# TinyMPC/TinyMPC

Hardware: AMD Instinct MI355X
Metric: QP solves/sec (+ ADMM iters/sec), 64k-batch quadrotor hover (higher is better)
Workload: dtype f64; 1 GPU; quadrotor_hovering (nx=12, nu=4, N=10), 65536 identical instances per GPU, closed-loop MPC steps from a cold start (BASELINE configs[1]); batch_per_gpu=65536, total_batch=65536, parallelism=batch-sharded x1, mpc_steps_per_launch=8, stats_exchange=none (one rank), launcher=plain process

## Files before the change

tinympc_amd/csrc/admm_kernel.hip.h:

```cpp
#pragma once
#include <hip/hip_runtime.h>
#include <stdint.h>

namespace tinympc_amd {

enum : int {
    TAB_MB = 0,
    TAB_MF1 = 256,
    TAB_MF2 = 512,
    TAB_PT = 768,
    TAB_VEC = 1024,
    TAB_BOUNDS = 1024 + 16 * 16,
};
enum : int {
    VEC_CB = 0,
    VEC_CF = 1,
    VEC_QR = 2,
    VEC_SMASK = 3,
    VEC_NIM = 4,
    VEC_SOCFLAG = 5,
    VEC_CONE_BASE = 6,
    VEC_CONE_MU = 7,
    VEC_LINFLAG = 9,
    VEC_TLINFLAG = 10,
// ... 133 lines not shown
        ring1<0, NA>(a0, srcA, mA);
        ring1<NA, NB>(a0, srcB, mB);
        return a0;
    } else {
        double a0 = init, a1 = 0.0;
        ring<MODE, 0, NA>(a0, a1, srcA, mA);
        ring<MODE, NA, NB>(a0, a1, srcB, mB);
        return a0 + a1;
    }
}
template <int MODE, int COL0, int NCOL>
__device__ __forceinline__ double ring_sum(double init, double src, const double* m) {
    if constexpr (MODE == 2) {
        double a0 = init;
        ring1<COL0, NCOL>(a0, src, m);
        return a0;
    } else {
        double a0 = init, a1 = 0.0;
        ring<MODE, COL0, NCOL>(a0, a1, src, m);
        return a0 + a1;
    }
}
template <int MODE, int COL0, int NCOL>
__device__ __forceinline__ double ring_short(double init, double src, const double* m) {
    if constexpr (MODE == 1) return ring_sum<1, COL0, NCOL>(init, src, m);
    else { double a0 = init; ring1<COL0, NCOL>(a0, src, m); return a0; }
}


#define RINGH_LO(k, p) DPP_FMA("a0", "src", "m" #k, "%[c0]+" #k, "0x3")
#define RINGH_HI(k, p) DPP_FMA("a0", "src", "m" #k, "8+%[c0]+" #k, "0xc")
#define RINGH_CASE(K)                                                                                                                    \
    if constexpr (NCOL == K)                                                                                                             \
        asm("s_nop 1\n\t" DPP_REP(K, RINGH_LO) "s_nop 0\n\t" DPP_REP(K, RINGH_HI) : [a0] "+&v"(a0) : [src] "v"(src), [c0] "i"(COL0) DPP_REP(K, DPP_ROW_M));
template <int COL0, int NCOL>
__device__ __forceinline__ void ring1_half(double& a0, double src, const double* m) {
    static_assert(NCOL >= 1 && COL0 + NCOL <= 8, "one half row");
    RINGH_CASE(1) RINGH_CASE(2) RINGH_CASE(3) RINGH_CASE(4) RINGH_CASE(5) RINGH_CASE(6) RINGH_CASE(7) RINGH_CASE(8)
}


#if defined(TINYMPC_FUSED_NX) && defined(TINYMPC_FUSED_NU)
#define TINYMPC_FUSED 1
constexpr bool fused_shape(int na, int nb) { return na == TINYMPC_FUSED_NX && nb == TINYMPC_FUSED_NU; }
#define FUSED_ROW_OPERANDS [c0] "i"(TINYMPC_FUSED_NX) DPP_REP(TINYMPC_FUSED_NX, DPP_ROW_A) DPP_REP(TINYMPC_FUSED_NU, DPP_ROW_B)
#else
constexpr bool fused_shape(int, int) { return false; }
#endif
#define BWD_COL_A(k, p) DPP_FMA("acc", "sa", "a" #k, #k, "0xf")
#define BWD_COL_B(k, p) DPP_FMA("acc", "sb", "b" #k, "%[c0]+" #k, "0xf")
#define FWD_COL_A(k, p) DPP_FMA("t", "xi", "a" #k, #k, "0xf")
#define FWD_COL_B(k, p) DPP_FMA("xn", "t", "b" #k, "%[c0]+" #k, "0xf")
#define FWD_COL_B_INPLACE(k, p) DPP_FMA("t", "t", "b" #k, "%[c0]+" #k, "%[bm]")
template <int NA, int NB>
__device__ __forceinline__ void fused_backward_step(double& qlo, double& acc, double vn, double g, double qx, double rho, double smask, double cb,
                                                    double sa, double sb, const double* ma, const double* mb_) {
#ifdef TINYMPC_FUSED
    if constexpr (fused_shape(NA, NB)) {
        double tmp;
        asm("v_add_f64 %[tmp], %[vn], -%[g]\n\t"
            "v_fma_f64 %[qlo], -%[rho], %[tmp], %[qx]\n\t"
            "v_fma_f64 %[acc], %[qlo], %[smask], %[cb]\n\t"
            DPP_REP(TINYMPC_FUSED_NX, BWD_COL_A) DPP_REP(TINYMPC_FUSED_NU, BWD_COL_B)
            : [qlo] "=&v"(qlo), [acc] "=&v"(acc), [tmp] "=&v"(tmp)
            : [vn] "v"(vn), [g] "v"(g), [qx] "v"(qx), [rho] "v"(rho), [smask] "v"(smask), [cb] "v"(cb), [sa] "v"(sa), [sb] "v"(sb), FUSED_ROW_OPERANDS);
    }
#endif
}
template <int NA, int NB>
__device__ __forceinline__ void fused_backward_step_soc(double& qlo, double& acc, double vn, double g, double qx, double w, double rho,
                                                        double smask, double cb, double sa, double sb, const double* ma, const double* mb_) {
#ifdef TINYMPC_FUSED
    if constexpr (fused_shape(NA, NB)) {
        double tmp;
        asm("v_add_f64 %[tmp], %[vn], -%[g]\n\t"
            "v_fma_f64 %[qlo], -%[rho], %[tmp], %[qx]\n\t"
            "v_fma_f64 %[qlo], -%[rho], %[w], %[qlo]\n\t"
            "v_fma_f64 %[acc], %[qlo], %[smask], %[cb]\n\t"
            DPP_REP(TINYMPC_FUSED_NX, BWD_COL_A) DPP_REP(TINYMPC_FUSED_NU, BWD_COL_B)
            : [qlo] "=&v"(qlo), [acc] "=&v"(acc), [tmp] "=&v"(tmp)
            : [vn] "v"(vn), [g] "v"(g), [qx] "v"(qx), [rho] "v"(rho), [smask] "v"(smask), [cb] "v"(cb), [sa] "v"(sa), [sb] "v"(sb),
              [w] "v"(w), FUSED_ROW_OPERANDS);
    }
#endif
}
template <int NA, int NB, bool INPLACE = false>
__device__ __forceinline__ void fused_forward_step(double& tt, double& vn, double& t, double& xn, double xi, double g, double lo, double hi,
                                                   const double* ma, const double* mb_) {
#ifdef TINYMPC_FUSED
    if constexpr (fused_shape(NA, NB) && !(INPLACE && TINYMPC_FUSED_NX % 4 == 0)) {
        double vm;
        asm("v_add_f64 %[tt], %[xi], %[g]\n\t"
            "v_max_f64 %[vm], %[lo], %[tt]\n\t"
            DPP_REP(TINYMPC_FUSED_NX, FWD_COL_A)
            "v_min_f64 %[vn], %[hi], %[vm]\n\t"
            "v_mov_b64 %[xn], %[t]\n\t"
            DPP_REP(TINYMPC_FUSED_NU, FWD_COL_B)
            : [tt] "=&v"(tt), [vm] "=&v"(vm), [vn] "=&v"(vn), [xn] "=&v"(xn), [t] "+&v"(t)
            : [xi] "v"(xi), [g] "v"(g), [lo] "v"(lo), [hi] "v"(hi), FUSED_ROW_OPERANDS);
    }
    if constexpr (fused_shape(NA, NB) && INPLACE && TINYMPC_FUSED_NX % 4 == 0) {
        asm("v_add_f64 %[tt], %[xi], %[g]\n\t"
            DPP_REP(TINYMPC_FUSED_NX, FWD_COL_A)
            "v_max_f64 %[vn], %[lo], %[tt]\n\t"
            "v_min_f64 %[vn], %[hi], %[vn]\n\t"
            DPP_REP(TINYMPC_FUSED_NU, FWD_COL_B_INPLACE)
            : [tt] "=&v"(tt), [vn] "=&v"(vn), [t] "+&v"(t)
            : [xi] "v"(xi), [g] "v"(g), [lo] "v"(lo), [hi] "v"(hi), [bm] "i"((1 << (TINYMPC_FUSED_NX / 4)) - 1), FUSED_ROW_OPERANDS);
        xn = t;
    }
#endif
}
#if defined(TINYMPC_FUSED) && TINYMPC_FUSED_NX + TINYMPC_FUSED_NU <= 8
#define TINYMPC_FUSED_HALF 1
#endif
#define HBWD_COL_A_LO(k, p) DPP_FMA("acc", "sa", "a" #k, #k, "0x3")
#define HBWD_COL_A_HI(k, p) DPP_FMA("acc", "sa", "a" #k, "8+" #k, "0xc")
#define HBWD_COL_B_LO(k, p) DPP_FMA("acc", "sb", "b" #k, "%[c0]+" #k, "0x3")
#define HBWD_COL_B_HI(k, p) DPP_FMA("acc", "sb", "b" #k, "8+%[c0]+" #k, "0xc")
#define HFWD_COL_A_LO(k, p) DPP_FMA("t", "xi", "a" #k, #k, "0x3")
#define HFWD_COL_A_HI(k, p) DPP_FMA("t", "xi", "a" #k, "8+" #k, "0xc")
#define HFWD_COL_B_LO(k, p) DPP_FMA("xn", "t", "b" #k, "%[c0]+" #k, "0x3")
#define HFWD_COL_B_HI(k, p) DPP_FMA("xn", "t", "b" #k, "8+%[c0]+" #k, "0xc")
template <int NA, int NB>
__device__ __forceinline__ void fused_backward_step_half(double& qlo, double& acc, double& dnp, double& tmpn, double tmp, double vnn, double gn, double qx,
                                                         double rho, double smask, double cb, double nim, double cf, double sa, double sb,
                                                         const double* ma, const double* mb_) {
#ifdef TINYMPC_FUSED_HALF
    if constexpr (fused_shape(NA, NB)) {
        asm("v_fma_f64 %[qlo], -%[rho], %[tmp], %[qx]\n\t"
            "v_fma_f64 %[acc], %[qlo], %[smask], %[cb]\n\t"
            "v_fma_f64 %[dnp], %[sa], %[nim], %[cf]\n\t"
            DPP_REP(TINYMPC_FUSED_NX, HBWD_COL_A_LO) DPP_REP(TINYMPC_FUSED_NU, HBWD_COL_B_LO)
            "v_add_f64 %[tmpn], %[vnn], -%[gn]\n\t"
            DPP_REP(TINYMPC_FUSED_NX, HBWD_COL_A_HI) DPP_REP(TINYMPC_FUSED_NU, HBWD_COL_B_HI)
            : [qlo] "=&v"(qlo), [acc] "=&v"(acc), [dnp] "=&v"(dnp), [tmpn] "=&v"(tmpn)
            : [tmp] "v"(tmp), [vnn] "v"(vnn), [gn] "v"(gn), [qx] "v"(qx), [rho] "v"(rho), [smask] "v"(smask), [cb] "v"(cb),
              [nim] "v"(nim), [cf] "v"(cf), [sa] "v"(sa), [sb] "v"(sb), FUSED_ROW_OPERANDS);
    }
#endif
}
template <int NA, int NB>
__device__ __forceinline__ void fused_forward_step_half(double& tt, double& vn, double& t, double& xn, double& gnew, double xi, double g,
                                                        double lo, double hi, const double* ma, const double* mb_) {
#ifdef TINYMPC_FUSED_HALF
    if constexpr (fused_shape(NA, NB)) {
        double vm;
        asm("v_add_f64 %[tt], %[xi], %[g]\n\t"
            "v_max_f64 %[vm], %[lo], %[tt]\n\t"
            DPP_REP(TINYMPC_FUSED_NX, HFWD_COL_A_LO)
            "v_min_f64 %[vn], %[hi], %[vm]\n\t"
            DPP_REP(TINYMPC_FUSED_NX, HFWD_COL_A_HI)
            "v_mov_b64 %[xn], %[t]\n\t"
            "v_add_f64 %[gnew], %[tt], -%[vn]\n\t"
            DPP_REP(TINYMPC_FUSED_NU, HFWD_COL_B_LO)
            "s_nop 0\n\t"
            DPP_REP(TINYMPC_FUSED_NU, HFWD_COL_B_HI)
            : [tt] "=&v"(tt), [vm] "=&v"(vm), [vn] "=&v"(vn), [xn] "=&v"(xn), [t] "+&v"(t), [gnew] "=&v"(gnew)
            : [xi] "v"(xi), [g] "v"(g), [lo] "v"(lo), [hi] "v"(hi), FUSED_ROW_OPERANDS);
    }
#endif
}

__device__ __forceinline__ double vmax64(double a, double b) {
    double r;
    asm("v_max_f64 %0, %1, %2" : "=v"(r) : "v"(a), "v"(b));
    return r;
}
__device__ __forceinline__ double vmin64(double a, double b) {
    double r;
    asm("v_min_f64 %0, %1, %2" : "=v"(r) : "v"(a), "v"(b));
    return r;
}
__device__ __forceinline__ double pinned_sub64(double a, double b) {
    double r = a - b;
    asm volatile("" : "+v"(r));
    return r;
}
__device__ __forceinline__ double vclamp64(double lo, double hi, double t) {
    double r;
    asm("v_max_f64 %0, %1, %2\n\tv_min_f64 %0, %3, %0" : "=&v"(r) : "v"(lo), "v"(t), "v"(hi));
    return r;
}

__device__ __forceinline__ double vmax_abs64(double a, double b) {
    double r;
    asm("v_max_f64 %0, %1, |%2|" : "=v"(r) : "v"(a), "v"(b));
    return r;
}
template <bool OPAQUE>
// ... 114 lines not shown

#ifndef TINYMPC_LIN_WAVES
#define TINYMPC_LIN_WAVES 0
#endif
constexpr long solve_kernel_lin_lds(int nx, int nu, int n, bool soc, int lin, int kmax, bool ub) {
    const int nz = nx + nu, csl = (nz + 1) | 1, cs = (nz + 1) | 1;
    return 8L * (nx * 16 + (ub ? 2 : 2 * n * 16) + ((lin & 1) ? 3 * kmax * 16 + 2 * 4 * n * csl : 0) +
                 ((lin & 2) ? 3 * n * kmax * 16 + 2 * 4 * n * csl : 0) + (soc ? (4 * n + 1) * 3 * cs : 0));
}
constexpr bool solve_kernel_lin_planes(int nx, int nu, int n, bool soc, int lin, int kmax, bool ub) {
    return lin != 0 && solve_kernel_lin_lds(nx, nu, n, soc, lin, kmax, ub) <= 64 * 1024 - 512;
}
constexpr int solve_kernel_lin_waves(int nx, int nu, int n, bool soc, int lin, int kmax, bool ub) {
    if (!solve_kernel_lin_planes(nx, nu, n, soc, lin, kmax, ub)) return 1;
    if (TINYMPC_LIN_WAVES > 0) return TINYMPC_LIN_WAVES;
    return (solve_kernel_waves_per_simd(nx + nu, n, soc) == 2 && 8 * solve_kernel_lin_lds(nx, nu, n, soc, lin, kmax, ub) <= 158 * 1024) ? 2 : 1;
}
template <int NF, int KMAX_, int LW_, int LPI_>
__device__ __forceinline__ void project_halfspace_columns(const int t, const int inst, const int n, const int csl, const int R0, const int S0,
                                                          double* pv, double* pg, const double* tab, const int tab_stride, const int nk) {
#pragma clang fp contract(off)
    for (int c = S0 + t; c < n; c += LPI_) {
        const int at = (inst * n + c) * csl + R0;
        const double* tk = tab + c * tab_stride;
        double z[NF], t0[NF];
#pragma unroll
        for (int r = 0; r < NF; ++r) { z[r] = pv[at + r]; t0[r] = z[r]; }
        for (int k = 0; k < nk; ++k) {
            double cv = 0.0;
#pragma unroll
            for (int r = 0; r < NF; ++r) { const double pr = tk[k * LW_ + R0 + r] * z[r]; cv = cv + pr; }
            const double bk = tk[KMAX_ * LW_ + k * LW_ + R0];
            if (cv > bk) {
                const double dist = (cv - bk) / tk[2 * KMAX_ * LW_ + k * LW_ + R0];
#pragma unroll
                for (int r = 0; r < NF; ++r) { const double pr = dist * tk[k * LW_ + R0 + r]; z[r] = z[r] - pr; }
            }
        }
#pragma unroll
        for (int r = 0; r < NF; ++r) { pv[at + r] = z[r]; pg[at + r] = t0[r] - z[r]; }
    }
}

template <int NX, int NU, int N, bool SOC, bool DBG, int MODE, int LIN = 0, bool HET = false, int KMAX = LIN_KMAX, bool ADAPT = false, bool UB = false, bool HALF = false,
          bool PF = false>
__global__ __launch_bounds__(64)
__attribute__((amdgpu_waves_per_eu(LIN != 0 ? solve_kernel_lin_waves(NX, NU, N, SOC, LIN, KMAX, UB) : solve_kernel_waves_per_simd(NX + NU, N, SOC, false, ADAPT),
                                   LIN != 0 ? solve_kernel_lin_waves(NX, NU, N, SOC, LIN, KMAX, UB) : solve_kernel_waves_per_simd(NX + NU, N, SOC, false, ADAPT))))
void admm_solve_kernel(const SolveArgs P) {
    constexpr bool LS = (LIN & 1) != 0, LT = (LIN & 2) != 0;
    constexpr int NZ = NX + NU;
    static_assert(NZ <= 16, "one instance per 16-lane DPP row");
    constexpr bool FUSED = MODE == 2 && LIN == 0 && fused_shape(NX, NU);
    static_assert(!HALF || (NZ <= 8 && FUSED && !SOC && !DBG && !HET && !ADAPT), "half rows: nx+nu <= 8, the plain box kernel on its fused step blocks");
    static_assert(!PF || (MODE == 2 && !SOC && !DBG && LIN == 0 && !HET && !ADAPT), "prefetch form: the plain box kernel");
    constexpr int RL = HALF ? 8 : 16;
    constexpr int IPW = 64 / RL;
    constexpr int RECD = N * NZ;
    constexpr int PF_PIECES = (IPW * RECD * 8 + 1023) / 1024;
    constexpr int PF_ARR = PF_PIECES * 128;
    constexpr unsigned long long RMASK = HALF ? 0xFFull : 0xFFFFull;
    const int lane = threadIdx.x & 63;
    const int j = lane & (RL - 1);
    const int grp = lane / RL;
    const bool is_state = j < NX;
    const bool is_input = (j >= NX) && (j < NZ);

    __shared__ double sPt[NX * 16];
    __shared__ double sLo[UB ? 1 : N * 16];
    __shared__ double sHi[UB ? 1 : N * 16];
    __shared__ double sLin[LS ? 3 * KMAX * 16 : 1];
    __shared__ double sTLin[LT ? 3 * N * KMAX * 16 : 1];
#ifndef TINYMPC_SOC_PD
#define TINYMPC_SOC_PD 2
#endif
    constexpr int SPD = TINYMPC_SOC_PD, SPR = SPD + 1;
    constexpr int CS = SOC ? ((NZ + 1) | 1) : 1;
    constexpr int SLOT_D = 3 * CS;
    constexpr int PL_GC = CS, PL_VC = 2 * CS;
    __shared__ double sC[SOC ? (4 * N + 1) * SLOT_D : 1];
    __shared__ double sP[ADAPT ? 4 * NX * NX : 1];
    constexpr int AKC = NX > NU ? NX : NU;
    constexpr bool HA = HET && ADAPT;
    __shared__ double sTab[(ADAPT && !HET) ? 3 * 16 * AKC : 1];
    __shared__ double sDl[ADAPT ? 4 * ADAPT_LOG : 1];
    if constexpr (ADAPT && !HET)
        for (int e = lane; e < 3 * 16 * AKC; e += 64) {
            const int t = e / (16 * AKC), r = e % (16 * AKC);
            sTab[e] = P.atab[t * 256 + (r % AKC) * 16 + r / AKC];
        }
    if constexpr (LS) for (int e = lane; e < 3 * KMAX * 16; e += 64) sLin[e] = P.tab[TAB_BOUNDS + 2 * N * 16 + e];
    if constexpr (LT) for (int e = lane; e < 3 * N * KMAX * 16; e += 64) sTLin[e] = P.tab[TAB_BOUNDS + 2 * N * 16 + 3 * KMAX * 16 + e];
    for (int e = lane; e < NX * 16; e += 64) sPt[e] = P.tab[TAB_PT + e];
    for (int e = lane; e < N * 16; e += 64) {
        if constexpr (!UB) {
            sLo[e] = P.tab[TAB_BOUNDS + e];
            sHi[e] = P.tab[TAB_BOUNDS + N * 16 + e];
        }
    }
    double mb[NZ], mf1[NX], mf2[NU];
#pragma unroll
    for (int k = 0; k < NZ; ++k) mb[k] = P.tab[TAB_MB + k * 16 + j];
#pragma unroll
    for (int k = 0; k < NX; ++k) mf1[k] = P.tab[TAB_MF1 + k * 16 + j];
#pragma unroll
    for (int k = 0; k < NU; ++k) mf2[k] = P.tab[TAB_MF2 + (NX + k) * 16 + j];
// ... 256 lines not shown
                if constexpr (LT) {
                    const double vt0 = (warm && tlin_lane) ? (resumed ? P.tlslack : P.prim)[off] : 0.0;
                    const double gt0 = (warm && tlin_lane) ? P.tldual[off] : 0.0;
                    if constexpr (LTP) { sTV[cl + s * CSL] = vt0; sTG[cl + s * CSL] = gt0; } else { VT[s] = vt0; GT[s] = gt0; }
                }
                if constexpr (DBG) { Qd[s] = 0.0; Pd[s] = 0.0; Dd[s] = 0.0; }
            }
            double x0v = x0v_in;
            auto terminal_term = [&]() {
                double pt[NX];
#pragma unroll
                for (int k = 0; k < NX; ++k)
                    pt[k] = ADAPT ? sP[grp * NX * NX + k + NX * (is_state ? j : 0)] : (HET ? het[TAB_PT + k * 16 + j] : sPt[k * 16 + j]);
                double xp = 0.0;
                if constexpr (HALF) ring1_half<0, NX>(xp, ref_last, pt);
                else xp = ring_sum<MODE, 0, NX>(0.0, ref_last, pt);
                qx_last_plain = QX[N - 1];
                QX[N - 1] = is_state ? -xp : QX[N - 1];
            };
            int ndl = 0;
            auto flush_c = [&](int n) {
                __builtin_amdgcn_fence(__ATOMIC_RELEASE, "wavefront");
                __builtin_amdgcn_wave_barrier();
                if (P.aC2 && is_state) {
                    double* c2 = P.aC2 + (size_t)b * (NX * NX) + NX * j;
                    double v[NX], d[NX];
#pragma unroll
                    for (int k = 0; k < NX; ++k) { v[k] = c2[k]; d[k] = P.atab[(HA ? (size_t)b * ATAB_DOUBLES : (size_t)0) + ATAB_DC2 + k * 16 + j]; }
                    for (int i = 0; i < n; ++i) {
                        const double dl = sDl[grp * ADAPT_LOG + i];
#pragma unroll
                        for (int k = 0; k < NX; ++k) v[k] = taylor_step(v[k], dl, d[k]);
                    }
#pragma unroll
                    for (int k = 0; k < NX; ++k) c2[k] = v[k];
                }
                if (P.aC1 && j < NU) {
                    double* c1 = P.aC1 + (size_t)b * (NU * NU) + NU * j;
                    double v[NU], d[NU];
#pragma unroll
                    for (int k = 0; k < NU; ++k) { v[k] = c1[k]; d[k] = P.atab[(HA ? (size_t)b * ATAB_DOUBLES : (size_t)0) + ATAB_DC1 + k * 16 + j]; }
                    for (int i = 0; i < n; ++i) {
                        const double dl = sDl[grp * ADAPT_LOG + i];
#pragma unroll
                        for (int k = 0; k < NU; ++k) v[k] = taylor_step(v[k], dl, d[k]);
                    }
#pragma unroll
                    for (int k = 0; k < NU; ++k) c1[k] = v[k];
                }
            };
            if (!has_traj && !(PF && P.ref_shared)) terminal_term();
            const int traj_k0 = has_traj ? (P.traj_step0 + (P.traj_offsets ? P.traj_offsets[b] : 0)) : 0;

            int iter = 0, solved = 0, checked = 0;
            unsigned acc_iter = 0, acc_solved = 0;
            bool vp_touched = false;
            double rp = 0.0, rd = 0.0;
            const int nsteps = PF ? 1 : (P.steps > 1 ? P.steps : 1);
            const int iter_first = resumed ? P.iter_base : 0;
            for (int step = 0; step < nsteps; ++step) {
                X[0] = x0v;
                if (has_traj) {
                    if (is_state) {
#pragma unroll
                        for (int s = 0; s < N; ++s) {
                            int kk = traj_k0 + step + s;
                            kk = kk < P.traj_points ? kk : P.traj_points - 1;
                            const double r = P.traj[(size_t)kk * NX + j];
                            QX[s] = -(r * qr);
                            if (s == N - 1) ref_last = r;
                        }
                    }
                    terminal_term();
                }
                if (P.reset_duals) {
#pragma unroll
                    for (int s = 0; s < N; ++s) G[s] = 0.0;
                }
                if constexpr (SOC) {
                    if (step > 0) {
#pragma unroll
                        for (int s = 0; s < N; ++s) {
                            const double vc0 = soc_lane ? X[s] : 0.0;
                            sC[cw + s * SLOT_D] = vc0 - sC[cw + s * SLOT_D + PL_GC];
                            sC[cw + s * SLOT_D + PL_VC] = vc0;
                        }
                    }
                }
                if constexpr (LS) {
                    if (step > 0) {
#pragma unroll
                        for (int s = 0; s < N; ++s) { if constexpr (LSP) sLV[cl + s * CSL] = lin_lane ? X[s] : 0.0; else VL[s] = lin_lane ? X[s] : 0.0; }
                    } else if (is_state && lin_lane && !resumed) { if constexpr (LSP) sLV[cl] = x0v; else VL[0] = x0v; }
                }
                if constexpr (LT) {
                    if (step > 0) {
#pragma unroll
                        for (int s = 0; s < N; ++s) { if constexpr (LTP) sTV[cl + s * CSL] = tlin_lane ? X[s] : 0.0; else VT[s] = tlin_lane ? X[s] : 0.0; }
                    } else if (is_state && tlin_lane && !resumed) { if constexpr (LTP) sTV[cl] = x0v; else VT[0] = x0v; }
                }
                if constexpr (LPL) __builtin_amdgcn_fence(__ATOMIC_RELEASE, "wavefront");
                const int iter0 = iter_first;
                iter = iter0; solved = 0;
                if (resumed && P.check_termination > 0) checked = 1;
                int countdown = P.check_termination;
                double wr[SOC ? SPR : 1];
                bool gcz[SOC_PASSES];
#pragma unroll
                for (int p = 0; p < SOC_PASSES; ++p) gcz[p] = false;
                if constexpr (SOC) {
#pragma unroll
                    for (int d = 1; d <= SPR && d <= N; ++d) wr[(N - d) % SPR] = sC[cw + (N - d) * SLOT_D];
                }
                for (int it = iter0; it < P.max_iter; ++it) {
                    double lvr[LSP ? SPR : 1], lgr[LSP ? SPR : 1], tvr[LTP ? SPR : 1], tgr[LTP ? SPR : 1];
                    if constexpr (LPL) {
#pragma unroll
                        for (int d = 1; d <= SPR && d <= N; ++d) {
                            if constexpr (LSP) { lvr[(N - d) % SPR] = sLV[cl + (N - d) * CSL]; lgr[(N - d) % SPR] = sLG[cl + (N - d) * CSL]; }
                            if constexpr (LTP) { tvr[(N - d) % SPR] = sTV[cl + (N - d) * CSL]; tgr[(N - d) % SPR] = sTG[cl + (N - d) * CSL]; }
                        }
                    }
                    auto lin_w = [&](const int s_) { if constexpr (LSP) return lvr[s_ % SPR] - lgr[s_ % SPR]; else return VL[LSR ? s_ : 0] - GL[LSR ? s_ : 0]; };
                    auto tlin_w = [&](const int s_) { if constexpr (LTP) return tvr[s_ % SPR] - tgr[s_ % SPR]; else return VT[LTR ? s_ : 0] - GT[LTR ? s_ : 0]; };
                    double qhi;
                    {
                        double t = fma(-rho, VN[N - 1] - G[N - 1], QX[N - 1]);
                        if constexpr (SOC) t = fma(-rho, wr[(N - 1) % SPR], t);
                        if constexpr (LS) t = fma(-rho, lin_w(N - 1), t);
                        if constexpr (LT) t = fma(-rho, tlin_w(N - 1), t);
                        qhi = t;
                        if constexpr (DBG) {
                            double ql = fma(-rho, VN[N - 1] - G[N - 1], qx_last_plain);
                            if constexpr (SOC) ql = fma(-rho, wr[(N - 1) % SPR], ql);
                            if constexpr (LS) ql = fma(-rho, lin_w(N - 1), ql);
                            if constexpr (LT) ql = fma(-rho, tlin_w(N - 1), ql);
                            Qd[N - 1] = is_state ? ql : t;
                            Pd[N - 1] = t;
                        }
                    }
                    double pcur = qhi;
                    if constexpr (HALF) {
                        double tmpv = VN[N - 2] - G[N - 2];
#pragma unroll
                        for (int i = N - 2; i >= 0; --i) {
                            double qlo, res, dnp, tmpn;
                            constexpr int dummy = 0;
                            const int in = i > 0 ? i - 1 : dummy;
                            fused_backward_step_half<NX, NU>(qlo, res, dnp, tmpn, tmpv, VN[in], G[in], QX[i], rho, smask, cb, nim, cf, pcur, qhi, mb, mb + NX);
                            if (i + 1 <= N - 2) Dn[i + 1] = dnp;
                            tmpv = tmpn;
                            pcur = res;
                            qhi = qlo;
                        }
                        Dn[0] = fma(pcur, nim, cf);
                    }
#pragma unroll
                    for (int i = N - 2; i >= 0 && !HALF; --i) {
                        if constexpr (SOC) {
                            if (i >= SPD) wr[(i - SPD) % SPR] = sC[cw + (i - SPD) * SLOT_D];
                        }
                        if constexpr (LSP) { if (i >= SPD) { lvr[(i - SPD) % SPR] = sLV[cl + (i - SPD) * CSL]; lgr[(i - SPD) % SPR] = sLG[cl + (i - SPD) * CSL]; } }
                        if constexpr (LTP) { if (i >= SPD) { tvr[(i - SPD) % SPR] = sTV[cl + (i - SPD) * CSL]; tgr[(i - SPD) % SPR] = sTG[cl + (i - SPD) * CSL]; } }
                        if constexpr (SOC || LPL) __builtin_amdgcn_sched_barrier(0);
                        if constexpr (FUSED) {
                            double qlo, res;
                            if constexpr (SOC) fused_backward_step_soc<NX, NU>(qlo, res, VN[i], G[i], QX[i], wr[i % SPR], rho, smask, cb, pcur, qhi, mb, mb + NX);
                            else fused_backward_step<NX, NU>(qlo, res, VN[i], G[i], QX[i], rho, smask, cb, pcur, qhi, mb, mb + NX);
                            pcur = res;
                            Dn[i] = fma(res, nim, cf);
                            if constexpr (DBG) { Qd[i] = qlo; Pd[i] = res; Dd[i + 1] = res; }
                            qhi = qlo;
                            continue;
                        }
                        double qlo = fma(-rho, VN[i] - G[i], QX[i]);
                        if constexpr (SOC) qlo = fma(-rho, wr[i % SPR], qlo);
                        if constexpr (LS) qlo = fma(-rho, lin_w(i), qlo);
                        if constexpr (LT) qlo = fma(-rho, tlin_w(i), qlo);
                        const double res = ring_sum2<MODE, NX, NU>(fma(qlo, smask, cb), pcur, mb, qhi, mb + NX);
                        pcur = res;
                        Dn[i] = fma(res, nim, cf);
                        if constexpr (DBG) { Qd[i] = qlo; Pd[i] = res; Dd[i + 1] = res; }
                        qhi = qlo;
                    }
                    constexpr bool LAZY_RES = N <= 12;
                    constexpr bool TIGHT = FUSED && !HALF && LAZY_RES && !SOC && NX % 4 == 0;
                    double pmax = 0.0, dmax = 0.0;
                    auto slot_update = [&](const int s, const double lo, const double hi, const double gcv, const double glv, const double gtv) {
                        const double xi = X[s];
                        const double t = xi + G[s];
                        const double vn = TIGHT ? vclamp64(lo, hi, t) : vmin64(hi, vmax64(lo, t));
                        if constexpr (!LAZY_RES) {
                            pmax = resid_max<true>(pmax, xi - vn);
                            dmax = resid_max<true>(dmax, VP[s] - vn);
                        }
                        G[s] = t - vn;
                        VN[s] = vn;
                        if constexpr (SOC) {
                            sC[cw + s * SLOT_D] = fma(xi, socmask, gcv);
                        }
                        if constexpr (LSP) sLV[cl + s * CSL] = (lin_lane && (is_state || s >= 1)) ? (xi + glv) : 0.0;
                        if constexpr (LTP) sTV[cl + s * CSL] = (tlin_lane && (is_state || s >= 1)) ? (xi + gtv) : 0.0;
                        if constexpr (LSR || LTR) {
                            auto halfspaces = [&](double z, const double* tabk, const int nk) {
                                for (int k = 0; k < nk; ++k) {
                                    const double a = tabk[k * 16 + j];
                                    const double bk = tabk[KMAX * 16 + k * 16 + j];
                                    const double nn = tabk[2 * KMAX * 16 + k * 16 + j];
                                    const double prod = a * z;
                                    double cs = 0.0, ci = 0.0;
                                    ring1<0, NX>(cs, prod, ones);
                                    ring1<NX, NU>(ci, prod, ones);
                                    const double cv = is_state ? cs : ci;
                                    if (cv > bk) z = z - ((cv - bk) / nn) * a;
                                }
                                return z;
                            };
                            if constexpr (LSR) {
                                const bool on = lin_lane && (is_state || s >= 1);
                                double vl = on ? (xi + GL[s]) : 0.0;
                                vl = halfspaces(vl, sLin, P.n_lin);
// ... 37 lines not shown
                            const double xi = X[i];
                            if constexpr (HALF) {
                                double gnew;
                                fused_forward_step_half<NX, NU>(tt, vn, t, xn, gnew, xi, G[i], lo_c, hi_c, mf1, mf2);
                                X[i + 1] = xn;
                                if constexpr (!LAZY_RES) {
                                    pmax = resid_max<true>(pmax, xi - vn);
                                    dmax = resid_max<true>(dmax, VP[i] - vn);
                                }
                                G[i] = gnew;
                                VN[i] = vn;
                                lo_c = lo_n; hi_c = hi_n;
                                continue;
                            }
                            fused_forward_step<NX, NU, TIGHT>(tt, vn, t, xn, xi, G[i], lo_c, hi_c, mf1, mf2);
                            X[i + 1] = xn;
                            if constexpr (!LAZY_RES) {
                                pmax = resid_max<true>(pmax, xi - vn);
                                dmax = resid_max<true>(dmax, VP[i] - vn);
                            }
                            if constexpr (TIGHT) {
                                __builtin_amdgcn_sched_barrier(0);
                                if (i > 0) G[i - 1] = pinned_sub64(tt_d, vn_d);
                                tt_d = tt; vn_d = vn;
                            } else G[i] = tt - vn;
                            VN[i] = vn;
                            if constexpr (SOC) sC[cw + i * SLOT_D] = fma(xi, socmask, gr[i % SPR]);
                            lo_c = lo_n; hi_c = hi_n;
                            continue;
                        }
                        const double t = ring_sum<MODE, 0, NX>(Dn[i], X[i], mf1);
                        X[i + 1] = ring_short<MODE, NX, NU>(t, t, mf2);
                        slot_update(i, lo_c, hi_c, gr[SOC ? i % SPR : 0], glr[LSP ? i % SPR : 0], gtr[LTP ? i % SPR : 0]);
                        lo_c = lo_n; hi_c = hi_n;
                    }
                    if constexpr (TIGHT && N >= 2) G[N - 2] = tt_d - vn_d;
                    (void)tt_d; (void)vn_d;
                    slot_update(N - 1, lo_c, hi_c, gr[SOC ? (N - 1) % SPR : 0], glr[LSP ? (N - 1) % SPR : 0], gtr[LTP ? (N - 1) % SPR : 0]);
                    if constexpr (LPL) {
                        __builtin_amdgcn_fence(__ATOMIC_RELEASE, "wavefront");
                        __builtin_amdgcn_wave_barrier();
                        if constexpr (LSP) {
                            if (lin_x_on) project_halfspace_columns<NX, KMAX, 16, 16>(j, grp, N, CSL, 0, 0, sLV, sLG, sLin, 0, P.n_lin);
                            if (lin_u_on) project_halfspace_columns<NU, KMAX, 16, 16>(j, grp, N, CSL, NX, 1, sLV, sLG, sLin, 0, P.n_lin);
                        }
                        if constexpr (LTP) {
                            if (tlin_x_on) project_halfspace_columns<NX, KMAX, 16, 16>(j, grp, N, CSL, 0, 0, sTV, sTG, sTLin, 3 * KMAX * 16, P.n_tlin);
                            if (tlin_u_on) project_halfspace_columns<NU, KMAX, 16, 16>(j, grp, N, CSL, NX, 1, sTV, sTG, sTLin, 3 * KMAX * 16, P.n_tlin);
                        }
                        __builtin_amdgcn_fence(__ATOMIC_RELEASE, "wavefront");
                        __builtin_amdgcn_wave_barrier();
                    }
                    bool conv = false;
                    auto termination = [&]() {
                        if (countdown > 0 && --countdown == 0) {
                            countdown = P.check_termination;
                            checked = 1;
                            constexpr int PS0 = N >= 2 ? 1 : 0, PS1 = N - 1;
                            auto lost = [&](const int s) {
                                return (int)(fabs(X[s] - VN[s]) >= P.tol_pri) | (int)(fabs(VP[s] - VN[s]) * rho >= P.tol_dua);
                            };
                            const bool maybe = ((int)!(rho > 0.0) | (int)!(lost(PS0) | lost(PS1))) != 0;
                            unsigned long long fold = __ballot(maybe);
                            fold &= fold >> 1; fold &= fold >> 2; fold &= fold >> 4;
                            if constexpr (!HALF) fold &= fold >> 8;
                            const bool any_row = (fold & (HALF ? 0x0101010101010101ull : 0x0001000100010001ull)) != 0ull;
                            const bool last_test = (P.max_iter - 1 - it) < P.check_termination;
                            if (last_test || any_row) {
                                if constexpr (LAZY_RES) {
#pragma unroll
                                    for (int s = 0; s < N; ++s) {
                                        pmax = resid_max<false>(pmax, X[s] - VN[s]);
                                        dmax = resid_max<false>(dmax, VP[s] - VN[s]);
                                    }
                                }
                                rp = pmax;
                                rd = dmax * rho;
                                const bool ok = (rp < P.tol_pri) && (rd < P.tol_dua);
                                const unsigned long long bal = __ballot(ok);
                                conv = ((bal >> (grp * RL)) & RMASK) == RMASK;
                            }
                        }
                    };
                    if constexpr (SOC) {
                        __builtin_amdgcn_fence(__ATOMIC_RELEASE, "wavefront");
                        __builtin_amdgcn_wave_barrier();
                        double n0 = sC[item_at[0]], n1 = sC[item_at[0] + 1], n2 = sC[item_at[0] + 2];
#pragma unroll
                        for (int d = 1; d <= SPR && d <= N; ++d) wr[(N - d) % SPR] = sC[cw + (N - d) * SLOT_D];
                        termination();
                        bool any_exact = false;
#pragma unroll
                        for (int p = 0; p < SOC_PASSES; ++p) {
                            if (p > 0 && p >= soc_passes) break;
                            const int at = item_at[p];
                            if (p > 0) { n0 = sC[at]; n1 = sC[at + 1]; n2 = sC[at + 2]; }
                            const double s0 = n0, s1 = n1, s2 = n2;
                            if (soc_all_inside(s0, s1, s2, item_mu[p])) {
                                sC[at + PL_VC] = s0; sC[at + PL_VC + 1] = s1; sC[at + PL_VC + 2] = s2;
                                if (!gcz[p]) {
                                    sC[at + PL_GC] = 0.0; sC[at + PL_GC + 1] = 0.0; sC[at + PL_GC + 2] = 0.0;
                                    gcz[p] = true;
                                }
                            } else {
                                double r0, r1, r2;
                                soc_project3(s0, s1, s2, item_mu[p], item_rmu[p], mu_pow2, r0, r1, r2);
                                const double g0 = s0 - r0, g1 = s1 - r1, g2 = s2 - r2;
                                sC[at + PL_VC] = r0; sC[at + PL_VC + 1] = r1; sC[at + PL_VC + 2] = r2;
                                sC[at + PL_GC] = g0; sC[at + PL_GC + 1] = g1; sC[at + PL_GC + 2] = g2;
                                sC[at] = r0 - g0; sC[at + 1] = r1 - g1; sC[at + 2] = r2 - g2;
                                gcz[p] = false;
                                any_exact = true;
                            }
                        }
                        if (it == iter0 && !proj_lane) {
#pragma unroll
                            for (int s = 0; s < N; ++s) sC[cw + s * SLOT_D + PL_GC] = 0.0;
                        }
                        __builtin_amdgcn_fence(__ATOMIC_RELEASE, "wavefront");
                        __builtin_amdgcn_wave_barrier();
                        if (any_exact) {
#pragma unroll
                            for (int d = 1; d <= SPR && d <= N; ++d) wr[(N - d) % SPR] = sC[cw + (N - d) * SLOT_D];
                        }
                    }
                    iter += 1;
                    if constexpr (ADAPT) {
                        if (it > 0 && it % 5 == 0) {
                            double at[NX];
#pragma unroll
                            for (int k = 0; k < NX; ++k) at[k] = HA ? atab_i[ATAB_AT + k * 16 + j] : sTab[j * AKC + k];
                            double pri_res = 0.0, ax_max = 0.0, z_max = 0.0, dual_res = 0.0, px_max = 0.0, aty_max = 0.0, q_max = 0.0;
                            double pxq_max = 0.0;
#pragma unroll
                            for (int i = 0; i < N - 1; ++i) {
                                const double axs = ring_sum<MODE, 0, NX>(0.0, X[i], mf1);
                                const double dyn = ring_short<MODE, NX, NU>(axs, is_input ? X[i + 1] : 0.0, mf2) - X[i + 1];
                                const double a = is_state ? dyn : X[i + 1];
                                const double zz = VN[i + 1];
                                const bool on = is_state || is_input;
                                pri_res = fmax(pri_res, on ? fabs(a - zz) : 0.0);
                                ax_max = fmax(ax_max, on ? fabs(a) : 0.0);
                                z_max = fmax(z_max, on ? fabs(zz) : 0.0);
                                const double init = is_state ? (i >= 1 ? -G[i] : 0.0) : G[i + 1];
                                const double aty = ring_sum<MODE, 0, NX>(init, G[i + 1], at);
                                const double xs = is_state ? X[i] : X[i + 1];
                                const double px = qr * xs;
                                dual_res = fmax(dual_res, on ? fabs((px + px) + aty) : 0.0);
                                pxq_max = fmax(pxq_max, on ? fabs(px) : 0.0);
                                aty_max = fmax(aty_max, on ? fabs(aty) : 0.0);
                            }
                            {
                                double prow[NX];
#pragma unroll
                                for (int k = 0; k < NX; ++k) prow[k] = sP[grp * NX * NX + (is_state ? j : 0) + NX * k];
                                const double pxl = ring_sum<MODE, 0, NX>(0.0, X[N - 1], prow);
                                const double ql = qr * X[N - 1];
                                const double atyl = -G[N - 1];
                                dual_res = fmax(dual_res, is_state ? fabs((pxl + ql) + atyl) : 0.0);
                                px_max = fmax(pxq_max, is_state ? fabs(pxl) : 0.0);
                                aty_max = fmax(aty_max, is_state ? fabs(atyl) : 0.0);
                                q_max = fmax(pxq_max, is_state ? fabs(ql) : 0.0);
                            }
                            pri_res = grp_max16(pri_res); ax_max = grp_max16(ax_max); z_max = grp_max16(z_max);
                            dual_res = grp_max16(dual_res); px_max = grp_max16(px_max); aty_max = grp_max16(aty_max); q_max = grp_max16(q_max);
                            const double pri_norm = fmax(ax_max, z_max);
                            const double dual_norm = fmax(fmax(px_max, aty_max), q_max);
                            const double eps = 1e-10;
                            const double normalized_pri = pri_res / (pri_norm + eps);
                            const double normalized_dual = dual_res / (dual_norm + eps);
                            const double ratio = normalized_pri / (normalized_dual + eps);
                            double new_rho = rho * sqrt(ratio);
                            if (P.aclip) new_rho = fmin(fmax(new_rho, P.arho_min), P.arho_max);
                            const double delta = new_rho - rho;
                            if (is_state) {
#pragma unroll
                                for (int k = 0; k < NU; ++k) mb[NX + k] = -taylor_step(-mb[NX + k], delta, (HA ? atab_i[ATAB_DK + k * 16 + j] : sTab[(16 + j) * AKC + k]));
#pragma unroll
                                for (int k = 0; k < NX; ++k) {
                                    const int e = grp * NX * NX + k + NX * j;
                                    sP[e] = taylor_step(sP[e], delta, (HA ? atab_i[ATAB_DP + k * 16 + j] : sTab[(32 + j) * AKC + k]));
                                }
                            } else if (is_input) {
#pragma unroll
                                for (int k = 0; k < NX; ++k) mf1[k] = -taylor_step(-mf1[k], delta, (HA ? atab_i[ATAB_DK + k * 16 + j] : sTab[(16 + j) * AKC + k]));
                            }
                            if (P.aC1 || P.aC2) {
                                if (j == 0) sDl[grp * ADAPT_LOG + ndl] = delta;
                                if (++ndl == ADAPT_LOG) { flush_c(ndl); ndl = 0; }
                            }
                            rho = new_rho;
                            __builtin_amdgcn_fence(__ATOMIC_RELEASE, "wavefront");
                            __builtin_amdgcn_wave_barrier();
                            QX[N - 1] = qx_last_plain;
                            terminal_term();
                        }
                    }
                    if constexpr (!SOC) termination();
                    if (conv) { solved = 1; break; }
#pragma unroll
                    for (int s = 0; s < N; ++s) VP[s] = VN[s];
                    vp_touched = true;
                }
                acc_iter += (unsigned)(iter - iter0);
                acc_solved += (unsigned)solved;
                if (P.iter_log && j == 0) P.iter_log[(size_t)step * P.batch + b] = solved ? iter : -iter;
                if (P.u0_log && is_input) P.u0_log[((size_t)step * P.batch + b) * NU + (j - NX)] = X[1];
                if (nsteps > 1) {
                    x0v = is_state ? X[1] : 0.0;
                }
            }

            constexpr bool FLS = TINYMPC_FULL_LINE_STORES != 0 && (PF || TINYMPC_FULL_LINE_STORES == 2) && !SOC && LIN == 0 && !DBG;
            if (FLS && (P.store_mask & 32) == 0) {
                if constexpr (FLS) {
                    const size_t seg = (size_t)b * (N * NZ) + j;
                    const bool in_row = j < NZ;
#pragma unroll
                    for (int s = 0; s < N; ++s) {
                        const size_t off = seg + s * NZ;
                        const double xs = is_input ? (s + 1 < N ? X[s + 1 < N ? s + 1 : s] : 0.0) : X[s];
                        const double vs = is_input ? (s + 1 < N ? VN[s + 1 < N ? s + 1 : s] : 0.0) : VN[s];
                        const double gs = is_input ? (s + 1 < N ? G[s + 1 < N ? s + 1 : s] : 0.0) : G[s];
                        const double ps = is_input ? (s + 1 < N ? VP[s + 1 < N ? s + 1 : s] : 0.0) : VP[s];
                        if (in_row) {
                            if (P.store_mask & 1) {
                                if (acc_iter > 0) { if constexpr (PF) P.prim[off] = xs; else store_primal(P.prim + off, xs); }
                                else if (s == 0 && is_state) P.prim[off] = xs;
                            }
                            if (P.store_mask & 2) P.slack[off] = vs;
                            if (P.store_mask & 4) P.dual[off] = gs;
                            if ((P.store_mask & 8) && vp_touched) P.slack_prev[off] = ps;
                        }
                    }
                }
            } else
#pragma unroll
            for (int s = 0; s < N; ++s) {
                const bool valid = is_state || (is_input && s >= 1);
                const size_t off = lbase + s * NZ;
                if (valid) {
                    if (((P.store_mask & 1) || ((P.store_mask & 32) && s <= 1)) && (acc_iter > 0 || (s == 0 && is_state))) {
                        if constexpr (SOC || LIN != 0) P.prim[off] = X[s];
                        else store_primal(P.prim + off, X[s]);
                    }
                    if (P.store_mask & 2) P.slack[off] = VN[s];
                    if (P.store_mask & 4) P.dual[off] = G[s];
                    if ((P.store_mask & 8) && vp_touched) P.slack_prev[off] = VP[s];
                    if constexpr (SOC) {
                        if (soc_lane && (P.store_mask & 16)) {
                            P.cslack[off] = sC[cw + s * SLOT_D + ((proj_lane || iter <= iter_first) ? PL_VC : 0)];
                            P.cdual[off] = sC[cw + s * SLOT_D + PL_GC];
                        }
                    }
                    if constexpr (LSP) { if (lin_lane && (P.store_mask & 16)) { P.lslack[off] = sLV[cl + s * CSL]; P.ldual[off] = sLG[cl + s * CSL]; } }
                    if constexpr (LTP) { if (tlin_lane && (P.store_mask & 16)) { P.tlslack[off] = sTV[cl + s * CSL]; P.tldual[off] = sTG[cl + s * CSL]; } }
                    if constexpr (LSR) { if (lin_lane && (P.store_mask & 16)) { P.lslack[off] = VL[s]; P.ldual[off] = GL[s]; } }
                    if constexpr (LTR) { if (tlin_lane && (P.store_mask & 16)) { P.tlslack[off] = VT[s]; P.tldual[off] = GT[s]; } }
                    if constexpr (DBG) {
                        if (P.dbg_qr && acc_iter > 0) {
                            P.dbg_qr[off] = Qd[s];
                            P.dbg_pd[off] = is_state ? Pd[s] : Dd[s];
                        }
                    }
                }
            }
            if constexpr (ADAPT) {
                if (ndl > 0) flush_c(ndl);
                if (j == 0) P.arho[b] = rho;
                if (is_state) {
#pragma unroll
                    for (int k = 0; k < NU; ++k) P.aK[(size_t)b * (NU * NX) + k + NU * j] = -mb[NX + k];
#pragma unroll
                    for (int k = 0; k < NX; ++k) P.aP[(size_t)b * (NX * NX) + k + NX * j] = sP[grp * NX * NX + k + NX * j];
                }
            }
            if (P.x0_next && acc_iter > 0 && is_state) P.x0_next[(size_t)b * NX + j] = X[1];
            const double ps = grp_maxw<RL>(is_state ? rp : 0.0), pi = grp_maxw<RL>(is_input ? rp : 0.0);
            const double ds = grp_maxw<RL>(is_state ? rd : 0.0), di = grp_maxw<RL>(is_input ? rd : 0.0);
            if (P.next_index) {
                const bool open = j == 0 && !solved;
                const unsigned long long m = __ballot(open);
                if (m) {
                    const int first = __ffsll((long long)m) - 1;
                    int at = 0;
                    if (lane == first) at = atomicAdd(P.next_count, __popcll(m));
                    at = __shfl(at, first);
                    if (open) P.next_index[at + __popcll(m & ((1ull << lane) - 1ull))] = b;
                }
            }
            if (j == 0) {
                P.status[b] = make_int4(iter, solved, solved ? 1 : 11, checked);
                double4 rr = make_double4(ps, pi, ds, di);
                *reinterpret_cast<double4*>(P.resid + (size_t)b * 4) = rr;
                if (P.accum) {
                    if constexpr (PF) {
                        __hip_atomic_fetch_add(&P.accum[b].x, acc_iter, __ATOMIC_RELAXED, __HIP_MEMORY_SCOPE_AGENT);
                        __hip_atomic_fetch_add(&P.accum[b].y, acc_solved, __ATOMIC_RELAXED, __HIP_MEMORY_SCOPE_AGENT);
                    } else {
                        uint2 ac = P.accum[b];
                        ac.x += acc_iter;
                        ac.y += acc_solved;
                        P.accum[b] = ac;
                    }
                }
            }
        }
    }
}

}
```

Before: 2.868 billion QP solves/s.

## Split termination check into staged ballots, scalar rho operand, derive iter counts after loop

The termination test now builds per-criterion wave ballots. When rho is uniform across the batch, a cheap dual check on one step gates the full primal and dual test. Rho is passed to the fused backward-step asm as an SGPR operand when uniform, which frees VGPRs and a move. Per-iteration bookkeeping (iter increment, solved/checked flags, vp_touched) is removed from the hot loop and reconstructed once after it exits. This trims scalar and vector work per ADMM iteration but makes the status bookkeeping more intricate. The half-row path now hardcodes an "s" constraint on rho, which requires rho to be wave-uniform there.

```diff
diff --git a/tinympc_amd/csrc/admm_kernel.hip.h b/tinympc_amd/csrc/admm_kernel.hip.h
--- a/tinympc_amd/csrc/admm_kernel.hip.h
+++ b/tinympc_amd/csrc/admm_kernel.hip.h
@@ -209,35 +209,41 @@
 #define FWD_COL_A(k, p) DPP_FMA("t", "xi", "a" #k, #k, "0xf")
 #define FWD_COL_B(k, p) DPP_FMA("xn", "t", "b" #k, "%[c0]+" #k, "0xf")
 #define FWD_COL_B_INPLACE(k, p) DPP_FMA("t", "t", "b" #k, "%[c0]+" #k, "%[bm]")
-template <int NA, int NB>
+template <int NA, int NB, bool RS = false>
 __device__ __forceinline__ void fused_backward_step(double& qlo, double& acc, double vn, double g, double qx, double rho, double smask, double cb,
                                                     double sa, double sb, const double* ma, const double* mb_) {
 #ifdef TINYMPC_FUSED
     if constexpr (fused_shape(NA, NB)) {
         double tmp;
-        asm("v_add_f64 %[tmp], %[vn], -%[g]\n\t"
-            "v_fma_f64 %[qlo], -%[rho], %[tmp], %[qx]\n\t"
-            "v_fma_f64 %[acc], %[qlo], %[smask], %[cb]\n\t"
-            DPP_REP(TINYMPC_FUSED_NX, BWD_COL_A) DPP_REP(TINYMPC_FUSED_NU, BWD_COL_B)
-            : [qlo] "=&v"(qlo), [acc] "=&v"(acc), [tmp] "=&v"(tmp)
-            : [vn] "v"(vn), [g] "v"(g), [qx] "v"(qx), [rho] "v"(rho), [smask] "v"(smask), [cb] "v"(cb), [sa] "v"(sa), [sb] "v"(sb), FUSED_ROW_OPERANDS);
+#define FUSED_BWD_STEP(RHO_CLASS)                                                                                                                \
+        asm("v_add_f64 %[tmp], %[vn], -%[g]\n\t"                                                                                                 \
+            "v_fma_f64 %[qlo], -%[rho], %[tmp], %[qx]\n\t"                                                                                       \
+            "v_fma_f64 %[acc], %[qlo], %[smask], %[cb]\n\t"                                                                                      \
+            DPP_REP(TINYMPC_FUSED_NX, BWD_COL_A) DPP_REP(TINYMPC_FUSED_NU, BWD_COL_B)                                                            \
+            : [qlo] "=&v"(qlo), [acc] "=&v"(acc), [tmp] "=&v"(tmp)                                                                               \
+            : [vn] "v"(vn), [g] "v"(g), [qx] "v"(qx), [rho] RHO_CLASS(rho), [smask] "v"(smask), [cb] "v"(cb), [sa] "v"(sa), [sb] "v"(sb), FUSED_ROW_OPERANDS)
+        if constexpr (RS) FUSED_BWD_STEP("s"); else FUSED_BWD_STEP("v");
+#undef FUSED_BWD_STEP
     }
 #endif
 }
-template <int NA, int NB>
+template <int NA, int NB, bool RS = false>
 __device__ __forceinline__ void fused_backward_step_soc(double& qlo, double& acc, double vn, double g, double qx, double w, double rho,
                                                         double smask, double cb, double sa, double sb, const double* ma, const double* mb_) {
 #ifdef TINYMPC_FUSED
     if constexpr (fused_shape(NA, NB)) {
         double tmp;
-        asm("v_add_f64 %[tmp], %[vn], -%[g]\n\t"
-            "v_fma_f64 %[qlo], -%[rho], %[tmp], %[qx]\n\t"
-            "v_fma_f64 %[qlo], -%[rho], %[w], %[qlo]\n\t"
-            "v_fma_f64 %[acc], %[qlo], %[smask], %[cb]\n\t"
-            DPP_REP(TINYMPC_FUSED_NX, BWD_COL_A) DPP_REP(TINYMPC_FUSED_NU, BWD_COL_B)
-            : [qlo] "=&v"(qlo), [acc] "=&v"(acc), [tmp] "=&v"(tmp)
-            : [vn] "v"(vn), [g] "v"(g), [qx] "v"(qx), [rho] "v"(rho), [smask] "v"(smask), [cb] "v"(cb), [sa] "v"(sa), [sb] "v"(sb),
-              [w] "v"(w), FUSED_ROW_OPERANDS);
+#define FUSED_BWD_STEP_SOC(RHO_CLASS)                                                                                                            \
+        asm("v_add_f64 %[tmp], %[vn], -%[g]\n\t"                                                                                                 \
+            "v_fma_f64 %[qlo], -%[rho], %[tmp], %[qx]\n\t"                                                                                       \
+            "v_fma_f64 %[qlo], -%[rho], %[w], %[qlo]\n\t"                                                                                        \
+            "v_fma_f64 %[acc], %[qlo], %[smask], %[cb]\n\t"                                                                                      \
+            DPP_REP(TINYMPC_FUSED_NX, BWD_COL_A) DPP_REP(TINYMPC_FUSED_NU, BWD_COL_B)                                                            \
+            : [qlo] "=&v"(qlo), [acc] "=&v"(acc), [tmp] "=&v"(tmp)                                                                               \
+            : [vn] "v"(vn), [g] "v"(g), [qx] "v"(qx), [rho] RHO_CLASS(rho), [smask] "v"(smask), [cb] "v"(cb), [sa] "v"(sa), [sb] "v"(sb),         \
+              [w] "v"(w), FUSED_ROW_OPERANDS)
+        if constexpr (RS) FUSED_BWD_STEP_SOC("s"); else FUSED_BWD_STEP_SOC("v");
+#undef FUSED_BWD_STEP_SOC
     }
 #endif
 }
@@ -292,7 +298,7 @@
             "v_add_f64 %[tmpn], %[vnn], -%[gn]\n\t"
             DPP_REP(TINYMPC_FUSED_NX, HBWD_COL_A_HI) DPP_REP(TINYMPC_FUSED_NU, HBWD_COL_B_HI)
             : [qlo] "=&v"(qlo), [acc] "=&v"(acc), [dnp] "=&v"(dnp), [tmpn] "=&v"(tmpn)
-            : [tmp] "v"(tmp), [vnn] "v"(vnn), [gn] "v"(gn), [qx] "v"(qx), [rho] "v"(rho), [smask] "v"(smask), [cb] "v"(cb),
+            : [tmp] "v"(tmp), [vnn] "v"(vnn), [gn] "v"(gn), [qx] "v"(qx), [rho] "s"(rho), [smask] "v"(smask), [cb] "v"(cb),
               [nim] "v"(nim), [cf] "v"(cf), [sa] "v"(sa), [sb] "v"(sb), FUSED_ROW_OPERANDS);
     }
 #endif
@@ -513,6 +519,7 @@
     constexpr int NZ = NX + NU;
     static_assert(NZ <= 16, "one instance per 16-lane DPP row");
     constexpr bool FUSED = MODE == 2 && LIN == 0 && fused_shape(NX, NU);
+    constexpr bool RHO_UNIFORM = !HET && !ADAPT;
     static_assert(!HALF || (NZ <= 8 && FUSED && !SOC && !DBG && !HET && !ADAPT), "half rows: nx+nu <= 8, the plain box kernel on its fused step blocks");
     static_assert(!PF || (MODE == 2 && !SOC && !DBG && LIN == 0 && !HET && !ADAPT), "prefetch form: the plain box kernel");
     constexpr int RL = HALF ? 8 : 16;
@@ -875,7 +882,8 @@
             if (!has_traj && !(PF && P.ref_shared)) terminal_term();
             const int traj_k0 = has_traj ? (P.traj_step0 + (P.traj_offsets ? P.traj_offsets[b] : 0)) : 0;
 
-            int iter = 0, solved = 0, checked = 0;
+            int iter = 0;
+            bool solved = false, checked = false;
             unsigned acc_iter = 0, acc_solved = 0;
             bool vp_touched = false;
             double rp = 0.0, rd = 0.0;
@@ -924,9 +932,9 @@
                 }
                 if constexpr (LPL) __builtin_amdgcn_fence(__ATOMIC_RELEASE, "wavefront");
                 const int iter0 = iter_first;
-                iter = iter0; solved = 0;
-                if (resumed && P.check_termination > 0) checked = 1;
+                if (resumed && P.check_termination > 0) checked = true;
                 int countdown = P.check_termination;
+                int left = 0;
                 double wr[SOC ? SPR : 1];
                 bool gcz[SOC_PASSES];
 #pragma unroll
@@ -988,8 +996,8 @@
                         if constexpr (SOC || LPL) __builtin_amdgcn_sched_barrier(0);
                         if constexpr (FUSED) {
                             double qlo, res;
-                            if constexpr (SOC) fused_backward_step_soc<NX, NU>(qlo, res, VN[i], G[i], QX[i], wr[i % SPR], rho, smask, cb, pcur, qhi, mb, mb + NX);
-                            else fused_backward_step<NX, NU>(qlo, res, VN[i], G[i], QX[i], rho, smask, cb, pcur, qhi, mb, mb + NX);
+                            if constexpr (SOC) fused_backward_step_soc<NX, NU, RHO_UNIFORM>(qlo, res, VN[i], G[i], QX[i], wr[i % SPR], rho, smask, cb, pcur, qhi, mb, mb + NX);
+                            else fused_backward_step<NX, NU, RHO_UNIFORM>(qlo, res, VN[i], G[i], QX[i], rho, smask, cb, pcur, qhi, mb, mb + NX);
                             pcur = res;
                             Dn[i] = fma(res, nim, cf);
                             if constexpr (DBG) { Qd[i] = qlo; Pd[i] = res; Dd[i + 1] = res; }
@@ -1133,33 +1141,41 @@
                         __builtin_amdgcn_wave_barrier();
                     }
                     bool conv = false;
+                    constexpr bool TWO_STAGE = LAZY_RES && !SOC && !DBG;
                     auto termination = [&]() {
                         if (countdown > 0 && --countdown == 0) {
                             countdown = P.check_termination;
-                            checked = 1;
                             constexpr int PS0 = N >= 2 ? 1 : 0, PS1 = N - 1;
-                            auto lost = [&](const int s) {
-                                return (int)(fabs(X[s] - VN[s]) >= P.tol_pri) | (int)(fabs(VP[s] - VN[s]) * rho >= P.tol_dua);
+                            auto pri_ok = [&](const int s) { return __builtin_amdgcn_ballot_w64(!(fabs(X[s] - VN[s]) >= P.tol_pri)); };
+                            auto dua_ok = [&](const int s) { return __builtin_amdgcn_ballot_w64(!(fabs(VP[s] - VN[s]) * rho >= P.tol_dua)); };
+                            auto any_row = [&](unsigned long long fold) {
+                                fold &= fold >> 1; fold &= fold >> 2; fold &= fold >> 4;
+                                if constexpr (!HALF) fold &= fold >> 8;
+                                return (fold & (HALF ? 0x0101010101010101ull : 0x0001000100010001ull)) != 0ull;
                             };
-                            const bool maybe = ((int)!(rho > 0.0) | (int)!(lost(PS0) | lost(PS1))) != 0;
-                            unsigned long long fold = __ballot(maybe);
-                            fold &= fold >> 1; fold &= fold >> 2; fold &= fold >> 4;
-                            if constexpr (!HALF) fold &= fold >> 8;
-                            const bool any_row = (fold & (HALF ? 0x0101010101010101ull : 0x0001000100010001ull)) != 0ull;
-                            const bool last_test = (P.max_iter - 1 - it) < P.check_termination;
-                            if (last_test || any_row) {
+                            bool full = (P.max_iter - 1 - it) < P.check_termination;
+                            if constexpr (RHO_UNIFORM) full = full || !(rho > 0.0);
+                            if (!full) {
+                                const unsigned long long no_rho = RHO_UNIFORM ? 0ull : __builtin_amdgcn_ballot_w64(!(rho > 0.0));
+                                if constexpr (TWO_STAGE) {
+                                    const unsigned long long m1 = dua_ok(PS0) | no_rho;
+                                    if (any_row(m1)) full = any_row(m1 & ((pri_ok(PS0) & dua_ok(PS1) & pri_ok(PS1)) | no_rho));
+                                } else full = any_row((dua_ok(PS0) & pri_ok(PS0) & dua_ok(PS1) & pri_ok(PS1)) | no_rho);
+                            }
+                            if (__builtin_expect(full, 0)) {
                                 if constexpr (LAZY_RES) {
 #pragma unroll
                                     for (int s = 0; s < N; ++s) {
-                                        pmax = resid_max<false>(pmax, X[s] - VN[s]);
-                                        dmax = resid_max<false>(dmax, VP[s] - VN[s]);
+                                        const bool ps = s == PS0 || s == PS1;
+                                        pmax = resid_max<false>(pmax, ps ? VN[s] - X[s] : X[s] - VN[s]);
+                                        dmax = resid_max<false>(dmax, ps ? VN[s] - VP[s] : VP[s] - VN[s]);
                                     }
                                 }
                                 rp = pmax;
                                 rd = dmax * rho;
-                                const bool ok = (rp < P.tol_pri) && (rd < P.tol_dua);
-                                const unsigned long long bal = __ballot(ok);
+                                const unsigned long long bal = __builtin_amdgcn_ballot_w64(rp < P.tol_pri) & __builtin_amdgcn_ballot_w64(rd < P.tol_dua);
                                 conv = ((bal >> (grp * RL)) & RMASK) == RMASK;
+                                if (conv) left = it + 1;
                             }
                         }
                     };
@@ -1205,7 +1221,6 @@
                             for (int d = 1; d <= SPR && d <= N; ++d) wr[(N - d) % SPR] = sC[cw + (N - d) * SLOT_D];
                         }
                     }
-                    iter += 1;
                     if constexpr (ADAPT) {
                         if (it > 0 && it % 5 == 0) {
                             double at[NX];
@@ -1278,11 +1293,14 @@
                         }
                     }
                     if constexpr (!SOC) termination();
-                    if (conv) { solved = 1; break; }
+                    if (conv) break;
 #pragma unroll
                     for (int s = 0; s < N; ++s) VP[s] = VN[s];
-                    vp_touched = true;
-                }
+                }
+                solved = left > 0;
+                iter = solved ? left : (iter0 < P.max_iter ? P.max_iter : iter0);
+                if (P.check_termination > 0 && iter - iter0 >= P.check_termination) checked = true;
+                if (iter - iter0 > (int)solved) vp_touched = true;
                 acc_iter += (unsigned)(iter - iter0);
                 acc_solved += (unsigned)solved;
                 if (P.iter_log && j == 0) P.iter_log[(size_t)step * P.batch + b] = solved ? iter : -iter;
@@ -1371,7 +1389,7 @@
                 }
             }
             if (j == 0) {
-                P.status[b] = make_int4(iter, solved, solved ? 1 : 11, checked);
+                P.status[b] = make_int4(iter, (int)solved, solved ? 1 : 11, (int)checked);
                 double4 rr = make_double4(ps, pi, ds, di);
                 *reinterpret_cast<double4*>(P.resid + (size_t)b * 4) = rr;
                 if (P.accum) {
```

New measurement: 2.863 billion QP solves/s. No clear change (-0.2%).
